# YaoChengTang/DecNet

Hardware: AMD Instinct MI355X
Metric: stereo pairs/sec at 960x540x192disp (hot path: stage-0 dense + SpaMat/SpaVar stages 1-3) (higher is better)
Workload: dtype f32 (bf16x3 on the bf16 matrix pipe); 1 GPU; BASELINE config 2: synthetic 960x540 (padded 972x540), max_disp 192->216: batch=8 synthetic pairs per GPU, feature maps of the 4-stage/scale-3 net, random-init CostRegNetNoDown(216); pairs_per_gpu=8, parallelism=dp1 (pairs sharded, all_gather of disparity maps)

## Files before the change

### decnet_amd/csrc/spamat_mfma.hip

```cpp
#include <stdlib.h>
#include <string.h>

#include <type_traits>

#include "common.h"


typedef float f32x4 __attribute__((ext_vector_type(4)));
typedef int i32x4 __attribute__((ext_vector_type(4)));
typedef __bf16 bf16x8 __attribute__((ext_vector_type(8)));

namespace {

enum { MODE_MAT = 0, MODE_VAR = 1, MODE_FUSED = 2 };

constexpr float NEG_BIG = -1.0e30f;
constexpr float LOG2E = 1.4426950408889634f;
constexpr int THREADS = 512, NWAVE = THREADS / 64;

__device__ __forceinline__ float fast_exp2(float x) { return __builtin_amdgcn_exp2f(x); }

__device__ __forceinline__ bool uniform_flag(bool f) { return __builtin_amdgcn_readfirstlane((int)f) != 0; }
template <bool SEL = true>
__device__ __forceinline__ float4 load4f(const float *__restrict__ safe, const float *__restrict__ row, int x, int W, bool ok) {
// ... 11 lines not shown
        if (x + 1 >= 0 && x + 1 < W) v.y = row[x + 1];
        if (x + 2 >= 0 && x + 2 < W) v.z = row[x + 2];
        if (x + 3 >= 0 && x + 3 < W) v.w = row[x + 3];
    }
    return v;
}
__device__ __forceinline__ float4 load4s(const float *__restrict__ row, int x, int W) {
    float4 v = make_float4(0.f, 0.f, 0.f, 0.f);
    if (x >= 0 && x < W) v.x = row[x];
    if (x + 1 >= 0 && x + 1 < W) v.y = row[x + 1];
    if (x + 2 >= 0 && x + 2 < W) v.z = row[x + 2];
    if (x + 3 >= 0 && x + 3 < W) v.w = row[x + 3];
    return v;
}

__device__ __forceinline__ int mask4_bits(const unsigned long long *__restrict__ rowbits, int x, int W) {
    if (x < 0 || x >= W) return 0;
    return (int)((rowbits[x >> 6] >> (x & 63)) & 15ull);
}

__device__ __forceinline__ int mask4_words(const unsigned *__restrict__ roww, int x, int W) {
    if (x < 0 || x >= W) return 0;
    return (int)((roww[x >> 5] >> (x & 31)) & 15u);
}

__device__ __forceinline__ void split3x8(const float (&x)[8], i32x4 &hi, i32x4 &mid, i32x4 &lo) {
    int h[8], m[8], l[8];
#pragma unroll
    for (int e = 0; e < 8; ++e) {
        h[e] = __float_as_int(x[e]) & 0xffff0000;
        const float r1 = x[e] - __int_as_float(h[e]);
        m[e] = __float_as_int(r1) & 0xffff0000;
        l[e] = __float_as_int(r1 - __int_as_float(m[e]));
    }
#pragma unroll
    for (int e = 0; e < 4; ++e) {
        hi[e] = __builtin_amdgcn_perm(h[2 * e + 1], h[2 * e], 0x07060302);
        mid[e] = __builtin_amdgcn_perm(m[2 * e + 1], m[2 * e], 0x07060302);
        lo[e] = __builtin_amdgcn_perm(l[2 * e + 1], l[2 * e], 0x07060302);
    }
}

__host__ __device__ inline int d16_pitch(int quads) { return quads + ((4 - quads) & 7); }
struct Layout {
    int SW, HALO, RP, Cq;
    int offR, offBX, offRK, offLM, offXL, offWT, total;
};
__host__ __device__ inline Layout make_layout(int C, int NT, int XT, bool d16 = false) {
    Layout l;
    l.SW = XT * 16;
    l.HALO = (NT - 1) * 16;
    l.Cq = (C + 3) & ~3;
    l.RP = ((l.HALO + l.SW + 31) & ~31) + 16;
    l.offR = 0;
    const int swh = ((XT + 1) / 2) * 16;
    const int rt = d16 ? 3 * ((C + 7) / 8) * 16 * (d16_pitch((l.HALO + swh) >> 2) + d16_pitch(swh >> 2)) : 0;
    l.offBX = l.offR + (l.Cq * l.RP > rt ? l.Cq * l.RP : rt);
    l.offRK = l.offBX + l.RP;
    l.offLM = l.offRK + l.RP + 4;
    l.offXL = l.offLM + l.SW + 16;
    l.offWT = l.offXL + l.SW;
    l.total = l.offWT + 32;
    return l;
}

__device__ __forceinline__ int wave_incl_scan(int v, int lane) {
#pragma unroll
    for (int o = 1; o < 64; o <<= 1) {
        int t = __shfl_up(v, o);
        if (lane >= o) v += t;
    }
    return v;
}

template <int M, int N, int STEP, class F>
__device__ __forceinline__ void live_tiles(int ntile, F &&f) {
    if constexpr (M < N) {
        if (STEP > 0 && M >= ntile) return;
        f(std::integral_constant<int, M>{});
        if constexpr (STEP == 2 && M + 1 < N) f(std::integral_constant<int, M + 1>{});
        live_tiles<M + (STEP > 1 ? STEP : 1), N, STEP>(ntile, f);
    }
}
template <int NTL, int MODE, int COMPACT>
__device__ __forceinline__ void softmax_passes(f32x4 (&acc)[NTL], int ntile, int D, int dl,
                                               const float *__restrict__ lds, int bias_off, int xr_off,
                                               int xlj, float mu_in,
                                               float &mx_o, float &S_o, float &mu_o, float &var_o,
                                               int m_lo = 0, int m_hi = 0) {
    constexpr int GS = COMPACT >= 2 ? 2 : COMPACT;
    int dlv = dl;
    asm volatile("" : "+v"(dlv));
    float mx0 = 0.000001f, mx1 = 0.000001f;
    (void)bias_off;
    int xo1 = xr_off;
    asm volatile("" : "+v"(xo1));
    const int *xp1 = reinterpret_cast<const int *>(lds) + xo1;
    const float xlf = (float)xlj, hD = 0.5f * (float)(D - 1), xlh = xlf - hD;
    live_tiles<0, NTL, GS>(ntile, [&](auto mc) {
        constexpr int m = decltype(mc)::value;
        {
            if (COMPACT >= 2) {
                if (COMPACT == 2 || m < m_lo || m >= m_hi) {
                    if (COMPACT == 3) asm volatile("" ::: "memory");
                    const float4 p = *reinterpret_cast<const float4 *>(xp1 + 16 * m);
                    acc[m][0] = fabsf(xlh - p.x) <= hD ? acc[m][0] : NEG_BIG;
                    acc[m][1] = fabsf(xlh - p.y) <= hD ? acc[m][1] : NEG_BIG;
                    acc[m][2] = fabsf(xlh - p.z) <= hD ? acc[m][2] : NEG_BIG;
                    acc[m][3] = fabsf(xlh - p.w) <= hD ? acc[m][3] : NEG_BIG;
                }
            } else if (COMPACT) {
                const int4 p = *reinterpret_cast<const int4 *>(xp1 + 16 * m);
                acc[m][0] = (unsigned)(xlj - p.x) < (unsigned)D ? acc[m][0] : NEG_BIG;
                acc[m][1] = (unsigned)(xlj - p.y) < (unsigned)D ? acc[m][1] : NEG_BIG;
                acc[m][2] = (unsigned)(xlj - p.z) < (unsigned)D ? acc[m][2] : NEG_BIG;
                acc[m][3] = (unsigned)(xlj - p.w) < (unsigned)D ? acc[m][3] : NEG_BIG;
            } else {
                if (m == 0 || 16 * m + 15 >= D) {
                    asm volatile("" ::: "memory");
#pragma unroll
                    for (int r = 0; r < 4; ++r) {
                        const int d = 16 * m + dlv - r;
                        acc[m][r] = (unsigned)d >= (unsigned)D ? NEG_BIG : acc[m][r];
                    }
                }
            }
            mx0 = fmaxf(fmaxf(mx0, acc[m][0]), acc[m][1]);
            mx1 = fmaxf(fmaxf(mx1, acc[m][2]), acc[m][3]);
        }
    });
    float mx = fmaxf(mx0, mx1);
    mx = fmaxf(mx, __shfl_xor(mx, 16));
    mx = fmaxf(mx, __shfl_xor(mx, 32));
    if (!COMPACT && MODE != MODE_MAT) {
        const float nmv = -mx * LOG2E;
        float Sa = 0.f, Sb = 0.f, T16a = 0.f, T16b = 0.f, Tt = 0.f;
#pragma unroll
        for (int m = 0; m < NTL; ++m) {
            if (m < ntile) {
                const float e0 = fast_exp2(fmaf(acc[m][0], LOG2E, nmv));
                const float e1 = fast_exp2(fmaf(acc[m][1], LOG2E, nmv));
                const float e2 = fast_exp2(fmaf(acc[m][2], LOG2E, nmv));
                const float e3 = fast_exp2(fmaf(acc[m][3], LOG2E, nmv));
                const float s4 = (e0 + e1) + (e2 + e3);
                const float t2 = fmaf(6.f, e3, fmaf(4.f, e2, e1 + e1));
                const float qq = fmaf(9.f, e3, fmaf(4.f, e2, e1));
                acc[m][0] = s4;
                acc[m][1] = t2;
                acc[m][2] = qq;
                if (m & 1) { Sb += s4; T16b = fmaf(s4, (float)(16 * m), T16b); }
                else { Sa += s4; T16a = fmaf(s4, (float)(16 * m), T16a); }
                Tt += t2;
            }
        }
        const float dlf = (float)dl;
        float Sl = Sa + Sb;
        float Tl = fmaf(dlf, Sl, fmaf(-0.5f, Tt, T16a + T16b));
        Sl += __shfl_xor(Sl, 16);
        Sl += __shfl_xor(Sl, 32);
        const float S = Sl + 0.000001f;
        float mu = mu_in;
        if (MODE != MODE_VAR) {
            Tl += __shfl_xor(Tl, 16);
            Tl += __shfl_xor(Tl, 32);
            mu = (Tl + 0.000001f) / S;
        }
        const float c0 = dlf - mu;
        float V0 = 0.f, V1 = 0.f;
#pragma unroll
        for (int m = 0; m < NTL; ++m) {
            if (m < ntile) {
                const float A = (float)(16 * m) + c0;
                const float u = fmaf(A, acc[m][0], -acc[m][1]);
                if (m & 1) V1 = fmaf(A, u, V1) + acc[m][2];
                else V0 = fmaf(A, u, V0) + acc[m][2];
            }
        }
        float Vl = V0 + V1;
        Vl += __shfl_xor(Vl, 16);
        Vl += __shfl_xor(Vl, 32);
        mx_o = mx; S_o = S; mu_o = mu; var_o = (Vl + 0.000001f) / S;
        return;
    }
    const float nm = -mx * LOG2E;
    float S0 = 0.f, S1 = 0.f, T0 = 0.f, T1 = 0.f;
    int xo2 = xr_off;
    asm volatile("" : "+v"(xo2));
    const int *xp2 = reinterpret_cast<const int *>(lds) + xo2;
    live_tiles<0, NTL, GS>(ntile, [&](auto mc) {
        constexpr int m = decltype(mc)::value;
        {
            int4 p;
            float4 pf;
            if (COMPACT >= 2) pf = *reinterpret_cast<const float4 *>(xp2 + 16 * m);
            else if (COMPACT) p = *reinterpret_cast<const int4 *>(xp2 + 16 * m);
#pragma unroll
            for (int r = 0; r < 4; r += 2) {
                float e0 = fast_exp2(fmaf(acc[m][r], LOG2E, nm));
                float e1 = fast_exp2(fmaf(acc[m][r + 1], LOG2E, nm));
                acc[m][r] = e0;
                acc[m][r + 1] = e1;
                S0 += e0;
                S1 += e1;
                if (MODE != MODE_VAR) {
                    if (COMPACT >= 2) {
                        T0 = fmaf(e0, xlf - (r == 0 ? pf.x : pf.z), T0);
                        T1 = fmaf(e1, xlf - (r == 0 ? pf.y : pf.w), T1);
                    } else if (COMPACT) {
                        T0 = fmaf(e0, (float)(xlj - (r == 0 ? p.x : p.z)), T0);
                        T1 = fmaf(e1, (float)(xlj - (r == 0 ? p.y : p.w)), T1);
                    } else {
                        T0 = fmaf(e0, (float)(16 * m - r), T0);
                        T1 = fmaf(e1, (float)(16 * m - r - 1), T1);
                    }
                }
            }
        }
    });
    const float dlf = (float)dl;
    float Sl = S0 + S1;
    float Tl = COMPACT ? T0 + T1 : fmaf(dlf, Sl, T0 + T1);
    Sl += __shfl_xor(Sl, 16);
    Sl += __shfl_xor(Sl, 32);
    const float S = Sl + 0.000001f;
    float mu = mu_in;
    if (MODE != MODE_VAR) {
        Tl += __shfl_xor(Tl, 16);
        Tl += __shfl_xor(Tl, 32);
        mu = (Tl + 0.000001f) / S;
    }
    float var = 0.f;
    if (MODE != MODE_MAT) {
        const float c0 = (COMPACT ? (float)xlj : dlf) - mu;
        float V0 = 0.f, V1 = 0.f;
        int xo3 = xr_off;
        asm volatile("" : "+v"(xo3));
        const int *xp3 = reinterpret_cast<const int *>(lds) + xo3;
        live_tiles<0, NTL, GS>(ntile, [&](auto mc) {
            constexpr int m = decltype(mc)::value;
            {
                int4 p;
                float4 pf;
                if (COMPACT >= 2) pf = *reinterpret_cast<const float4 *>(xp3 + 16 * m);
                else if (COMPACT) p = *reinterpret_cast<const int4 *>(xp3 + 16 * m);
#pragma unroll
                for (int r = 0; r < 4; r += 2) {
                    float d0, d1;
                    if (COMPACT >= 2) {
                        d0 = c0 - (r == 0 ? pf.x : pf.z);
                        d1 = c0 - (r == 0 ? pf.y : pf.w);
                    } else if (COMPACT) {
                        d0 = c0 - (float)(r == 0 ? p.x : p.z);
                        d1 = c0 - (float)(r == 0 ? p.y : p.w);
                    } else {
                        d0 = (float)(16 * m - r) + c0;
                        d1 = (float)(16 * m - r - 1) + c0;
                    }
                    V0 = fmaf(acc[m][r] * d0, d0, V0);
                    V1 = fmaf(acc[m][r + 1] * d1, d1, V1);
                }
            }
        });
        float Vl = V0 + V1;
        Vl += __shfl_xor(Vl, 16);
        Vl += __shfl_xor(Vl, 32);
        var = (Vl + 0.000001f) / S;
    }
    mx_o = mx; S_o = S; mu_o = mu; var_o = var;
}


__device__ __forceinline__ void dense16_loads8(float4 (&v)[8], const float *__restrict__ src, size_t plane, int g, int C,
                                               int x, int W, bool al) {
    if (al) {
        const bool whole = x + 3 < W;
#pragma unroll
        for (int c = 0; c < 8; ++c)
            v[c] = load4f<false>(src, src + (size_t)(8 * g + c) * plane, x, W, whole && 8 * g + c < C);
        __builtin_amdgcn_sched_barrier(0);
        if (__ballot(x < 0) != 0ull) {
#pragma unroll
            for (int c = 0; c < 8; ++c)
                if (x < 0) v[c] = make_float4(0.f, 0.f, 0.f, 0.f);
        }
        if (C & 7) {
#pragma unroll
            for (int c = 0; c < 8; ++c) {
                const bool ch = 8 * g + c < C;
                v[c] = make_float4(ch ? v[c].x : 0.f, ch ? v[c].y : 0.f, ch ? v[c].z : 0.f, ch ? v[c].w : 0.f);
            }
        }
        if ((W & 3) && x < W && !whole) {
#pragma unroll
            for (int c = 0; c < 8; ++c)
                v[c] = 8 * g + c < C ? load4s(src + (size_t)(8 * g + c) * plane, x, W) : make_float4(0.f, 0.f, 0.f, 0.f);
        }
    } else {
#pragma unroll
        for (int c = 0; c < 8; ++c)
            v[c] = 8 * g + c < C ? load4s(src + (size_t)(8 * g + c) * plane, x, W) : make_float4(0.f, 0.f, 0.f, 0.f);
    }
}

__device__ __forceinline__ void dense16_item_loads(float4 (&v)[8], int it, const float *__restrict__ lrow,
                                                   const float *__restrict__ rrow, size_t plane, int C, int W, int xs,
                                                   int SW, int HALO, int nRw) {
    const bool al = uniform_flag(((((uintptr_t)rrow) | ((uintptr_t)lrow) | ((uintptr_t)(plane * 4))) & 15) == 0);
    const int cg_n = (C + 7) >> 3, nqR = nRw >> 2, nqL = SW >> 2;
    const int nR_items = cg_n * nqR;
    const bool isL = it >= nR_items;
    const int k = isL ? it - nR_items : it, nq = isL ? nqL : nqR;
    const int g = k / nq, jq = k - g * nq;
    const float *src = isL ? lrow : rrow;
    const int x = isL ? xs + 4 * jq : xs - HALO + 4 * jq;
    dense16_loads8(v, src, plane, g, C, x, W, al);
}

template <int NT, int MODE, int CGT, bool PRE = false>
__device__ __forceinline__ void dense16_body(int *RT, const float *BX, const float *LM, const float *smem,
                                             const float *__restrict__ lrow, const float *__restrict__ rrow,
                                             const float *__restrict__ disparity, float *__restrict__ out,
                                             float *__restrict__ var_out, float *__restrict__ sum_sim,
                                             float *__restrict__ max_cost, size_t plane, size_t rowpix, int C, int W,
                                             int D, int xs, int XT, int SW, int HALO, int nRw, const float4 *pre = nullptr) {
    const int tid = threadIdx.x, lane = tid & 63, wave = tid >> 6;
    struct { int CG; } lo = {(C + 7) >> 3};
    const int PR = d16_pitch(nRw >> 2), PL = d16_pitch(SW >> 2);
    int *LT = RT + 3 * lo.CG * 16 * PR;
    {
        const bool al = uniform_flag(((((uintptr_t)rrow) | ((uintptr_t)lrow) | ((uintptr_t)(plane * 4))) & 15) == 0);
        const int cg_n = lo.CG, nqR = nRw >> 2, nqL = SW >> 2;
        const int nR_items = cg_n * nqR, n_items = nR_items + cg_n * nqL;
#pragma unroll 1
        for (int it = tid; it < n_items; it += THREADS) {
            const bool isL = it >= nR_items;
            const int k = isL ? it - nR_items : it, nq = isL ? nqL : nqR;
            const int g = k / nq, jq = k - g * nq;
            const float *src = isL ? lrow : rrow;
            const int x = isL ? xs + 4 * jq : xs - HALO + 4 * jq;
            float4 v[8];
            if (PRE && it == tid) {
#pragma unroll
                for (int c = 0; c < 8; ++c) v[c] = pre[c];
            } else {
                dense16_loads8(v, src, plane, g, C, x, W, al);
            }
            const int P = isL ? PL : PR;
            int *dst = (isL ? LT : RT) + (g * 4 * P + jq) * 4;
            const int tstride = cg_n * 16 * P;
#pragma unroll
            for (int pz = 0; pz < 4; ++pz) {
                float xv[8];
#pragma unroll
                for (int c = 0; c < 8; ++c) xv[c] = pz == 0 ? v[c].x : pz == 1 ? v[c].y : pz == 2 ? v[c].z : v[c].w;
                i32x4 th, tm, tl;
                split3x8(xv, th, tm, tl);
                *reinterpret_cast<i32x4 *>(dst + pz * 4 * P) = th;
                *reinterpret_cast<i32x4 *>(dst + tstride + pz * 4 * P) = tm;
                *reinterpret_cast<i32x4 *>(dst + 2 * tstride + pz * 4 * P) = tl;
            }
        }
    }
    __syncthreads();

    const int j = lane & 15, q = lane >> 4;
    const int dl = j - 4 * q;
    constexpr int CGB = CGT ? CGT : 1;
    const int cg_n = CGT ? CGT : lo.CG;
    const int tA_big = q >> 1, tA_small = q == 0 ? 0 : q == 2 ? 1 : 2;
    const int tB_big = q & 1, tB_small = q == 1 ? 0 : q == 3 ? 1 : 2;
    const int gsR = 16 * PR, gsL = 16 * PL;
    for (int xt = wave; xt < XT; xt += NWAVE) {
        const int x0 = xs + xt * 16;
        if (x0 >= W) break;
        const int x = x0 + j;
        const size_t pix = rowpix + x;
        const bool inside = x < W;
        const float rm = LM[xt * 16 + j];
        if (__ballot(rm != 0.f) == 0ull) {
            if (inside && q == 0) {
                if (MODE != MODE_VAR) out[pix] = 0.f;
                if (MODE != MODE_MAT) var_out[pix] = 0.f;
                sum_sim[pix] = 0.f;
                max_cost[pix] = 0.f;
            }
            continue;
        }
        f32x4 acc[NT];
#pragma unroll
        for (int m = 0; m < NT; ++m) {
            const float4 bz = *reinterpret_cast<const float4 *>(BX + (HALO + xt * 16) + 4 * q - 16 * m);
            acc[m] = f32x4{bz.x, bz.y, bz.z, bz.w};
        }
        const int sa = (j & 3) * PR + 4 * xt + (j >> 2), sb = (j & 3) * PL + 4 * xt + (j >> 2);
        const int *a_small = RT + (tA_small * cg_n * 4 * PR + sa) * 4;
        const int *a_big = RT + (tA_big * cg_n * 4 * PR + sa) * 4;
        const int *b_small = LT + (tB_small * cg_n * 4 * PL + sb) * 4;
        const int *b_big = LT + (tB_big * cg_n * 4 * PL + sb) * 4;
#pragma unroll
        for (int g = 0; g < CGB; ++g) {
            for (int gg = g; gg < cg_n; gg += CGB) {
                const i32x4 bs = *reinterpret_cast<const i32x4 *>(b_small + gg * gsL);
                const i32x4 bb = *reinterpret_cast<const i32x4 *>(b_big + gg * gsL);
#pragma unroll
                for (int m = 0; m < NT; ++m) {
                    const i32x4 av = *reinterpret_cast<const i32x4 *>(a_small + gg * gsR + (NT - 1 - m) * 16);
                    acc[m] = __builtin_amdgcn_mfma_f32_16x16x32_bf16(__builtin_bit_cast(bf16x8, av),
                                                                     __builtin_bit_cast(bf16x8, bs), acc[m], 0, 0, 0);
                }
#pragma unroll
                for (int m = 0; m < NT; ++m) {
                    const i32x4 av = *reinterpret_cast<const i32x4 *>(a_big + gg * gsR + (NT - 1 - m) * 16);
                    acc[m] = __builtin_amdgcn_mfma_f32_16x16x32_bf16(__builtin_bit_cast(bf16x8, av),
                                                                     __builtin_bit_cast(bf16x8, bb), acc[m], 0, 0, 0);
                }
            }
        }
        float mx, S, mu, var;
        const float mu_in = (MODE == MODE_VAR && inside) ? disparity[pix] : 0.f;
        softmax_passes<NT, MODE, 0>(acc, NT, D, dl, smem, 0, 0, 0, mu_in, mx, S, mu, var);
        if (inside && q == 0) {
            const bool on = rm != 0.f;
            if (MODE != MODE_VAR) out[pix] = on ? mu : 0.f;
            if (MODE != MODE_MAT) var_out[pix] = on ? var : 0.f;
            sum_sim[pix] = on ? S : 0.f;
            max_cost[pix] = on ? mx : 0.f;
        }
    }

}

template <int NT, int MODE, int KQ, int PPT, int NTHR, int CAP, int NTCMAX>
__device__ __forceinline__ int sparse_row_body(
    const float *__restrict__ ref, const float *__restrict__ tar, const float *__restrict__ rmask,
    const float *__restrict__ tmask, const float *__restrict__ disparity, float *__restrict__ out,
    float *__restrict__ var_out, float *__restrict__ sum_sim, float *__restrict__ max_cost, int C,
    int H, int W, int D, int row, int dense_pct, int mbits, int *fr_out = nullptr, int *fl_out = nullptr);
constexpr int MID_CAP = 640;

template <int NT, int MODE, int KQ, bool D16>
__device__ __forceinline__ void spamat_fwd_segment(
    const float *__restrict__ ref, const float *__restrict__ tar, const float *__restrict__ rmask,
    const float *__restrict__ tmask, const float *__restrict__ disparity, float *__restrict__ out,
    float *__restrict__ var_out, float *__restrict__ sum_sim, float *__restrict__ max_cost, int C,
    int H, int W, int D, int XT, int allow_compact, int marker, int seg, int row, int compact_pct, int mbits) {
    const float mark = marker ? sum_sim[(size_t)row * W + (size_t)seg * (XT * 16)] : -1.0f;
    if (marker && !(mark < 0.f))
        return;
    if constexpr (KQ == 2) {
        if (marker == 2 && mark == -2.0f) {
            if (sparse_row_body<NT, MODE, KQ, 4, THREADS, MID_CAP, NT + 1>(ref, tar, rmask, tmask, disparity, out, var_out,
                                                                          sum_sim, max_cost, C, H, W, D, row, 100,
                                                                          mbits) == 1)
                return;
            __syncthreads();
        }
    }
    extern __shared__ __attribute__((aligned(16))) float smem[];
    const Layout lo = make_layout(C, NT, XT, D16);
    float *Rs = smem + lo.offR;
    float *BX = smem + lo.offBX;
    int *XR = reinterpret_cast<int *>(BX);
    int *RK = reinterpret_cast<int *>(smem + lo.offRK);
    float *LM = smem + lo.offLM;
    int *RKL = reinterpret_cast<int *>(LM);
    int *XL = reinterpret_cast<int *>(smem + lo.offXL);
    int *WT = reinterpret_cast<int *>(smem + lo.offWT);
    const int SW = lo.SW, HALO = lo.HALO, RP = lo.RP;
    const int kq_n = KQ ? KQ : lo.Cq / 4;
    constexpr int KB = KQ ? KQ : 1;

    const int tid = threadIdx.x, lane = tid & 63, wave = tid >> 6;
    const int b = row / H, y = row - b * H;
    const int xs = seg * SW;
    const int nRw = HALO + SW;
    const size_t plane = (size_t)H * W;
    const float *lrow = ref + ((size_t)b * C * H + y) * W;
    const float *rrow = tar + ((size_t)b * C * H + y) * W;
    const float *trow = tmask + (size_t)row * W;
    const float *mrow = rmask + (size_t)row * W;
    const size_t rowpix = (size_t)row * W;
    const unsigned long long *tbits = reinterpret_cast<const unsigned long long *>(tmask) + (size_t)row * ((W + 63) >> 6);
    const unsigned long long *lbits = reinterpret_cast<const unsigned long long *>(rmask) + (size_t)row * ((W + 63) >> 6);

    unsigned mf_wr = 0, mf_wl = 0;
    if constexpr (D16) {
        if (mbits == 2) {
            const int q4 = tid * 4, xr_ = xs - HALO + q4, xl_ = xs + q4;
            const unsigned *hw = reinterpret_cast<const unsigned *>(max_cost + rowpix);
            mf_wr = hw[(q4 < nRw && xr_ >= 0 && xr_ < W) ? xr_ >> 5 : 0];
            mf_wl = hw[((W + 31) >> 5) + ((q4 < SW && xl_ < W) ? xl_ >> 5 : 0)];
        }
    }
    float4 d16_pre[D16 ? 8 : 1];
    if constexpr (D16) {
        const int xta = (XT + 1) / 2;
        const int n_items = ((C + 7) >> 3) * (((HALO + xta * 16) >> 2) + ((xta * 16) >> 2));
        if (tid < n_items) dense16_item_loads(d16_pre, tid, lrow, rrow, plane, C, W, xs, xta * 16, HALO, HALO + xta * 16);
    }
    const bool al_r = ((((uintptr_t)rrow) | ((uintptr_t)(plane * 4))) & 15) == 0;
    const int st_nq = nRw >> 2;
    const int st_rpp = THREADS / st_nq;
    const int st_r0 = tid / st_nq, st_jq = tid - st_r0 * st_nq;
    float4 st_v[D16 ? 1 : 8];
    float bfirst[(!D16 && KQ > 0) ? KQ : 1];
    if constexpr (!D16) {
        if (st_r0 < st_rpp) {
            const int x = xs - HALO + 4 * st_jq;
#pragma unroll
            for (int u = 0; u < 8; ++u) {
                const int c = st_r0 + u * st_rpp;
                st_v[u] = c < C ? load4_lanes(rrow + (size_t)c * plane, x, W, al_r) : make_float4(0.f, 0.f, 0.f, 0.f);
            }
        }
        if constexpr (KQ > 0) {
            const int jl = lane & 15, ql = lane >> 4;
            const int x = xs + wave * 16 + jl;
            const bool ok = wave < XT && x < W;
#pragma unroll
            for (int s = 0; s < KQ; ++s) bfirst[s] = (ok && 4 * s + ql < C) ? lrow[(size_t)(4 * s + ql) * plane + x] : 0.f;
        }
    }

    const int p4 = tid * 4;
    int fr = 0, fl = 0;
    {
        const bool alm = (((uintptr_t)trow) & 15) == 0 && (((uintptr_t)mrow) & 15) == 0;
        const bool almu = D16 && uniform_flag(alm && (W & 3) == 0);
        if (p4 < nRw) {
            const int x = xs - HALO + p4;
            if (mbits == 2) {
                if (D16) fr = (x >= 0 && x < W) ? (int)((mf_wr >> (x & 31)) & 15u) : 0;
                else fr = mask4_words(reinterpret_cast<const unsigned *>(max_cost + rowpix), x, W);
            } else if (mbits) {
                fr = mask4_bits(tbits, x, W);
            } else {
                float4 tv = almu ? load4f(trow, trow, x, W, true) : load4_lanes(trow, x, W, alm);
                fr = (tv.x != 0.f) | ((tv.y != 0.f) << 1) | ((tv.z != 0.f) << 2) | ((tv.w != 0.f) << 3);
            }
            float4 bv4;
            bv4.x = (fr & 1) ? 0.f : NEG_BIG;
            bv4.y = (fr & 2) ? 0.f : NEG_BIG;
            bv4.z = (fr & 4) ? 0.f : NEG_BIG;
            bv4.w = (fr & 8) ? 0.f : NEG_BIG;
            *reinterpret_cast<float4 *>(BX + p4) = bv4;
        }
        if (p4 < SW) {
            float4 mv;
            if (mbits) {
                if (D16 && mbits == 2) fl = (xs + p4 < W) ? (int)((mf_wl >> ((xs + p4) & 31)) & 15u) : 0;
                else fl = mbits == 2 ? mask4_words(reinterpret_cast<const unsigned *>(max_cost + rowpix) + ((W + 31) >> 5), xs + p4, W)
                                : mask4_bits(lbits, xs + p4, W);
                mv = make_float4((fl & 1) ? 1.f : 0.f, (fl & 2) ? 1.f : 0.f, (fl & 4) ? 1.f : 0.f, (fl & 8) ? 1.f : 0.f);
            } else {
                mv = almu ? load4f(mrow, mrow, xs + p4, W, true) : load4_lanes(mrow, xs + p4, W, alm);
                fl = (mv.x != 0.f) | ((mv.y != 0.f) << 1) | ((mv.z != 0.f) << 2) | ((mv.w != 0.f) << 3);
            }
            *reinterpret_cast<float4 *>(LM + p4) = mv;
        }
    }
    {
        const int ir = wave_incl_scan(__popc(fr), lane), il = wave_incl_scan(__popc(fl), lane);
        if (lane == 63) { WT[wave] = ir; WT[8 + wave] = il; }
    }

    int nR = 0, nL = 0;
    bool compact = false;
    if constexpr (D16) {
        __syncthreads();
#pragma unroll
        for (int w = 0; w < NWAVE; ++w) { nR += WT[w]; nL += WT[8 + w]; }
        const int validL = min(SW, W - xs);
        const int validR = min(W, xs + SW) - max(0, xs - HALO);
        compact = allow_compact && ((long)nL * nR * 100 < (long)validL * validR * compact_pct);
        if (!compact) {
            const int xta = (XT + 1) / 2, xtb = XT - xta;
            dense16_body<NT, MODE, (KQ + 1) / 2, true>(reinterpret_cast<int *>(Rs), BX, LM, smem, lrow, rrow, disparity, out,
                                                       var_out, sum_sim, max_cost, plane, rowpix, C, W, D, xs, xta, xta * 16,
                                                       HALO, HALO + xta * 16, d16_pre);
            if (xtb > 0 && xs + xta * 16 < W) {
                __syncthreads();
                dense16_body<NT, MODE, (KQ + 1) / 2>(reinterpret_cast<int *>(Rs), BX + xta * 16, LM + xta * 16, smem, lrow,
                                                     rrow, disparity, out, var_out, sum_sim, max_cost, plane, rowpix, C,
                                                     W, D, xs + xta * 16, xtb, xtb * 16, HALO, HALO + xtb * 16);
            }
            return;
        }
    }
    {
        const bool al = al_r;
        const int rpp = st_rpp;
        const int r0 = st_r0, jq = st_jq;
        if (r0 < rpp) {
            const int jj = 4 * jq, x = xs - HALO + jj;
            for (int c0 = r0; c0 < lo.Cq; c0 += 8 * rpp) {
                float4 v[8];
                if (!D16 && c0 == r0) {
#pragma unroll
                    for (int u = 0; u < 8; ++u) v[u] = st_v[D16 ? 0 : u];
                } else {
#pragma unroll
                    for (int u = 0; u < 8; ++u) {
                        const int c = c0 + u * rpp;
                        v[u] = c < C ? load4_lanes(rrow + (size_t)c * plane, x, W, al) : make_float4(0.f, 0.f, 0.f, 0.f);
                    }
                }
#pragma unroll
                for (int u = 0; u < 8; ++u) {
                    const int c = c0 + u * rpp;
                    if (c < lo.Cq) *reinterpret_cast<float4 *>(Rs + c * RP + jj) = v[u];
                }
            }
        }
        for (int c = tid; c < lo.Cq; c += THREADS) Rs[c * RP + RP - 1] = 0.f;
    }
    __syncthreads();

    const int validL = min(SW, W - xs);
    const int validR = min(W, xs + SW) - max(0, xs - HALO);
    if constexpr (!D16) {
#pragma unroll
        for (int w = 0; w < NWAVE; ++w) { nR += WT[w]; nL += WT[8 + w]; }
        compact = allow_compact && ((long)nL * nR * 100 < (long)validL * validR * compact_pct);
    }

    const int j = lane & 15, q = lane >> 4;

    if constexpr (!D16) if (!compact) {
        const int dl = j - 4 * q;
        float bv[KQ <= 6 ? KB : 1], bcur[KB];
        float rm = 0.f;
        auto fetch_left = [&](int xt, float (&dst)[KB]) {
            const int x = xs + xt * 16 + j;
            const bool ok = xt < XT && x < W;
            if (KQ) {
#pragma unroll
                for (int s = 0; s < KQ; ++s)
                    dst[s] = (ok && 4 * s + q < C) ? lrow[(size_t)(4 * s + q) * plane + x] : 0.f;
            }
        };
        constexpr bool PREF = KQ <= 6;
        if constexpr (PREF && KQ > 0) {
#pragma unroll
            for (int s = 0; s < KB; ++s) bv[s] = bfirst[s];
        } else if constexpr (PREF) {
            fetch_left(wave, bv);
        }
        for (int xt = wave; xt < XT; xt += NWAVE) {
            const int x0 = xs + xt * 16;
            if (x0 >= W) break;
            const int x = x0 + j;
            const size_t pix = rowpix + x;
            const bool inside = x < W;
            rm = LM[xt * 16 + j];
            if constexpr (PREF) {
#pragma unroll
                for (int s = 0; s < KB; ++s) bcur[s] = bv[s];
                fetch_left(xt + NWAVE, bv);
            } else if (KQ > 0 && xt == wave) {
#pragma unroll
                for (int s = 0; s < KB; ++s) bcur[s] = bfirst[KQ > 0 ? s : 0];
            } else {
                fetch_left(xt, bcur);
            }
            if (__ballot(rm != 0.f) == 0ull) {
                if (inside && q == 0) {
                    if (MODE != MODE_VAR) out[pix] = 0.f;
// ... 82 lines not shown
    while (S > 16 && (long)S * nL > 24L * validL) S >>= 1;
    __syncthreads();
    constexpr int NTC = NT + 1;
    while (S > 16) {
        int bad = 0;
        for (int g = tid; g * S < SW; g += THREADS) {
            const int jlo = max(0, g * S + HALO - (D - 1)), jhi = min(nRw - 1, g * S + HALO + S - 1);
            if (RK[jhi + 1] - RK[jlo] > 16 * NTC - 15) bad = 1;
        }
        if (!__syncthreads_or(bad)) break;
        S >>= 1;
    }

    for (int p = tid; p < validL; p += THREADS) {
        if (RKL[p + 1] == RKL[p]) {
            const size_t pix = rowpix + xs + p;
            if (MODE != MODE_VAR) out[pix] = 0.f;
            if (MODE != MODE_MAT) var_out[pix] = 0.f;
            sum_sim[pix] = 0.f;
            max_cost[pix] = 0.f;
        }
    }

    const int ngroups = (SW + S - 1) / S;
    for (int g = wave; g < ngroups; g += NWAVE) {
        const int gx = g * S;
        const int e0 = __builtin_amdgcn_readfirstlane(RKL[gx]), e1 = __builtin_amdgcn_readfirstlane(RKL[min(gx + S, SW)]);
        if (e1 == e0) continue;
        const int jlo = max(0, gx + HALO - (D - 1)), jhi = min(nRw - 1, gx + HALO + S - 1);
        const int r_lo = __builtin_amdgcn_readfirstlane(RK[jlo]), r_hi = __builtin_amdgcn_readfirstlane(RK[jhi + 1]);
        const int t0 = r_lo >> 4;
        const int ntile = r_hi > r_lo ? ((r_hi - 1) >> 4) - t0 + 1 : 0;
        for (int e = e0; e < e1; e += 16) {
            const bool act = e + j < e1;
            const int xl = XL[act ? e + j : e1 - 1];
            const int x = xs + xl;
            const size_t pix = rowpix + x;
            float bcur[KB];
            if (KQ) {
#pragma unroll
                for (int s = 0; s < KQ; ++s)
                    bcur[s] = (act && 4 * s + q < C) ? lrow[(size_t)(4 * s + q) * plane + x] : 0.f;
            }
            f32x4 acc[NTC];
            const int *xa = XR + 16 * t0 + j;
            live_tiles<0, NTC, 1>(ntile, [&](auto mc) {
                constexpr int m = decltype(mc)::value;
                {
                    const float *ap = Rs + q * RP + xa[16 * m];
                    f32x4 a4 = f32x4{0.f, 0.f, 0.f, 0.f};
                    if (KQ) {
#pragma unroll
                        for (int s = 0; s < KQ; ++s)
                            a4 = __builtin_amdgcn_mfma_f32_16x16x4f32(ap[4 * s * RP], bcur[s], a4, 0, 0, 0);
                    } else {
                        const float *bp = lrow + (size_t)q * plane + x;
                        for (int s = 0; s < kq_n; ++s) {
                            const float lv = (act && 4 * s + q < C) ? bp[(size_t)4 * s * plane] : 0.f;
                            a4 = __builtin_amdgcn_mfma_f32_16x16x4f32(ap[4 * s * RP], lv, a4, 0, 0, 0);
                        }
                    }
                    acc[m] = a4;
                }
            });
            float mx, Ssum, mu, var;
            const float mu_in = (MODE == MODE_VAR && act) ? disparity[pix] : 0.f;
            softmax_passes<NTC, MODE, 1>(acc, ntile, D, 0, smem, 0, lo.offBX + 16 * t0 + 4 * q, xl + HALO, mu_in,
                                         mx, Ssum, mu, var);
            if (act && q == 0) {
                if (MODE != MODE_VAR) out[pix] = mu;
                if (MODE != MODE_MAT) var_out[pix] = var;
                sum_sim[pix] = Ssum;
                max_cost[pix] = mx;
            }
        }
    }
}

template <int NT, int MODE, int KQ, bool D16>
__global__ __launch_bounds__(THREADS, (KQ > 6 ? 2 : 4)) void spamat_fwd_mfma(
    const float *__restrict__ ref, const float *__restrict__ tar, const float *__restrict__ rmask,
    const float *__restrict__ tmask, const float *__restrict__ disparity, float *__restrict__ out,
    float *__restrict__ var_out, float *__restrict__ sum_sim, float *__restrict__ max_cost, int C,
    int H, int W, int D, int segs_per_row, int XT, int allow_compact, int marker, int compact_pct, int mbits) {
    spamat_fwd_segment<NT, MODE, KQ, D16>(ref, tar, rmask, tmask, disparity, out, var_out, sum_sim, max_cost, C, H, W,
                                          D, XT, allow_compact, marker, blockIdx.x % segs_per_row,
                                          blockIdx.x / segs_per_row, compact_pct, mbits);
}

constexpr int SP_THREADS = 256, SP_CAP = 256;
constexpr size_t sparse_row_words(int kq, int ppt, int nthr, int cap) {
    return (size_t)(cap + 32) + 2 * (size_t)(nthr * ppt / 2 + 2) + cap + 32 + 2 * (size_t)4 * kq * (cap + 16);
}

template <int NT, int MODE, int KQ, int PPT, int NTHR, int CAP, int NTCMAX>
__device__ __forceinline__ int sparse_row_body(
    const float *__restrict__ ref, const float *__restrict__ tar, const float *__restrict__ rmask,
    const float *__restrict__ tmask, const float *__restrict__ disparity, float *__restrict__ out,
    float *__restrict__ var_out, float *__restrict__ sum_sim, float *__restrict__ max_cost, int C,
    int H, int W, int D, int row, int dense_pct, int mbits, int *fr_out, int *fl_out) {
    constexpr int CQ = 4 * KQ, NTC = NT + 1 < NTCMAX ? NT + 1 : NTCMAX;
    constexpr int SP_NWAVE_ = NTHR / 64, SP_FP_ = CAP + 16;
    extern __shared__ __attribute__((aligned(16))) float smem[];
    constexpr int NPX = NTHR * PPT, RKW = NPX / 2 + 2;
    constexpr int offXR = 0, offRK = CAP + 32, offRKL = offRK + RKW, offXL = offRKL + RKW,
                  offWT = offXL + CAP, offRF = offWT + 32, offLF = offRF + CQ * SP_FP_;
    float *XR = smem + offXR;
    unsigned short *RK = reinterpret_cast<unsigned short *>(smem + offRK);
    unsigned short *RKL = reinterpret_cast<unsigned short *>(smem + offRKL);
    int *XL = reinterpret_cast<int *>(smem) + offXL;
    int *WT = reinterpret_cast<int *>(smem) + offWT;
    float *RF = smem + offRF, *LF = smem + offLF;

    const int tid = threadIdx.x, lane = tid & 63, wave = tid >> 6;
    const int b = row / H, y = row - b * H;
    const size_t plane = (size_t)H * W, rowpix = (size_t)row * W;
    const float *lrow = ref + ((size_t)b * C * H + y) * W;
    const float *rrow = tar + ((size_t)b * C * H + y) * W;
    const float *trow = tmask + rowpix, *mrow = rmask + rowpix;

    constexpr bool ALL = CAP > 256 && PPT == 4;
    const int p4 = tid * PPT;
    float4 lv[ALL ? CQ : 1], rv[ALL ? CQ : 1];
    if constexpr (ALL) {
        const bool alf = ((W & 3) == 0) && ((((uintptr_t)lrow) | ((uintptr_t)rrow) | ((uintptr_t)(plane * 4))) & 15) == 0;
#pragma unroll
        for (int c = 0; c < CQ; ++c) {
            const bool ok = p4 < W && c < C;
            lv[c] = ok ? load4_lanes(lrow + (size_t)c * plane, p4, W, alf) : make_float4(0.f, 0.f, 0.f, 0.f);
            rv[c] = ok ? load4_lanes(rrow + (size_t)c * plane, p4, W, alf) : make_float4(0.f, 0.f, 0.f, 0.f);
        }
    }
    int fr = 0, fl = 0;
    {
        const bool alm = ((W & 3) == 0) && ((((uintptr_t)trow) | ((uintptr_t)mrow)) & 15) == 0;
#pragma unroll
        for (int u = 0; u < PPT; u += 4) {
            if (p4 + u < W) {
                if (mbits == 2) {
                    const unsigned *hw = reinterpret_cast<const unsigned *>(max_cost + rowpix);
                    fr |= mask4_words(hw, p4 + u, W) << u;
                    fl |= mask4_words(hw + ((W + 31) >> 5), p4 + u, W) << u;
                } else if (mbits) {
                    const int wpr = (W + 63) >> 6;
                    fr |= mask4_bits(reinterpret_cast<const unsigned long long *>(tmask) + (size_t)row * wpr, p4 + u, W) << u;
                    fl |= mask4_bits(reinterpret_cast<const unsigned long long *>(rmask) + (size_t)row * wpr, p4 + u, W) << u;
                } else {
                    const float4 tv = load4_lanes(trow, p4 + u, W, alm), mv = load4_lanes(mrow, p4 + u, W, alm);
                    fr |= ((tv.x != 0.f) | ((tv.y != 0.f) << 1) | ((tv.z != 0.f) << 2) | ((tv.w != 0.f) << 3)) << u;
                    fl |= ((mv.x != 0.f) | ((mv.y != 0.f) << 1) | ((mv.z != 0.f) << 2) | ((mv.w != 0.f) << 3)) << u;
                }
            }
        }
    }
    if (fr_out) { *fr_out = fr; *fl_out = fl; }
    const int cr = __popc(fr), cl = __popc(fl);
    const int ir = wave_incl_scan(cr, lane), il = wave_incl_scan(cl, lane);
    if (lane == 63) { WT[wave] = ir; WT[8 + wave] = il; }
    __syncthreads();
    int nR = 0, nL = 0, baseR = 0, baseL = 0;
#pragma unroll
    for (int w = 0; w < SP_NWAVE_; ++w) {
        if (w < wave) { baseR += WT[w]; baseL += WT[8 + w]; }
        nR += WT[w];
        nL += WT[8 + w];
    }
    nR = __builtin_amdgcn_readfirstlane(nR);
    nL = __builtin_amdgcn_readfirstlane(nL);
    if ((long)nL * nR * 100 >= (long)W * W * dense_pct) return 0;
    if (nL > CAP || nR > CAP) return (nL <= MID_CAP && nR <= MID_CAP) ? 2 : 0;
// ... 137 lines not shown
                if (MODE != MODE_VAR) *reinterpret_cast<float4 *>(out + pix) = make_float4(r[0][0], r[0][1], r[0][2], r[0][3]);
                if (MODE != MODE_MAT) *reinterpret_cast<float4 *>(var_out + pix) = make_float4(r[1][0], r[1][1], r[1][2], r[1][3]);
                *reinterpret_cast<float4 *>(sum_sim + pix) = make_float4(r[2][0], r[2][1], r[2][2], r[2][3]);
                *reinterpret_cast<float4 *>(max_cost + pix) = make_float4(r[3][0], r[3][1], r[3][2], r[3][3]);
            } else {
#pragma unroll
                for (int k = 0; k < 4; ++k) {
                    if (p4 + u + k < W) {
                        if (MODE != MODE_VAR) out[pix + k] = r[0][k];
                        if (MODE != MODE_MAT) var_out[pix + k] = r[1][k];
                        sum_sim[pix + k] = r[2][k];
                        max_cost[pix + k] = r[3][k];
                    }
                }
            }
        }
    }
    return 1;
}

template <int NT, int MODE, int KQ, int PPT>
__global__ __launch_bounds__(SP_THREADS, PPT == 4 ? 6 : 5) void spamat_fwd_sparse(
    const float *__restrict__ ref, const float *__restrict__ tar, const float *__restrict__ rmask,
    const float *__restrict__ tmask, const float *__restrict__ disparity, float *__restrict__ out,
    float *__restrict__ var_out, float *__restrict__ sum_sim, float *__restrict__ max_cost, int C,
    int H, int W, int D, int seg_w, int dense_pct, int mbits, int handover) {
    const int row = blockIdx.x;
    int fr = 0, fl = 0;
    const int rc = sparse_row_body<NT, MODE, KQ, PPT, SP_THREADS, SP_CAP, 8>(ref, tar, rmask, tmask, disparity, out, var_out,
                                                                            sum_sim, max_cost, C, H, W, D, row, dense_pct, mbits,
                                                                            &fr, &fl);
    if (rc != 1) {
        const size_t rowpix = (size_t)row * W;
        const float mark = rc == 2 ? -2.0f : -1.0f;
        for (int x = threadIdx.x * seg_w; x < W; x += SP_THREADS * seg_w) sum_sim[rowpix + x] = mark;
        if (handover) {
            extern __shared__ __attribute__((aligned(16))) float smem[];
            unsigned *wb = reinterpret_cast<unsigned *>(smem);
            const int nw = (W + 31) >> 5, p4 = threadIdx.x * PPT;
            __syncthreads();
            for (int i = threadIdx.x; i < 2 * nw; i += SP_THREADS) wb[i] = 0u;
            __syncthreads();
            if (p4 < W) {
                if (fr) atomicOr(&wb[p4 >> 5], (unsigned)fr << (p4 & 31));
                if (fl) atomicOr(&wb[nw + (p4 >> 5)], (unsigned)fl << (p4 & 31));
            }
            __syncthreads();
            for (int i = threadIdx.x; i < 2 * nw; i += SP_THREADS) reinterpret_cast<unsigned *>(max_cost + rowpix)[i] = wb[i];
        }
    }
}

template <int NT, int KQ>
int launch_nt(int mode, const float *ref, const float *tar, const float *rmask, const float *tmask,
              const float *disparity, float *out, float *var_out, float *sum_sim, float *max_cost,
              int B, int C, int H, int W, int D, int allow_compact, int mbits, hipStream_t stream) {
    const int xt_row = ceil_div(W, 16);
    static const int dense_fp32 = [] { const char *e = getenv("DECNET_SPAMAT_DENSE"); return e && !strcmp(e, "fp32"); }();
    const bool d16 = KQ == 2 && !dense_fp32;
    auto bytes = [&](int xt) { return (size_t)4 * make_layout(C, NT, xt, d16).total; };
    const size_t budget2 = (DECNET_LDS_BYTES - 2048) / 2, budget1 = DECNET_LDS_BYTES - 1024;
    int XT = xt_row > 64 ? ceil_div(xt_row, ceil_div(xt_row, 64)) : xt_row;
    if (bytes(XT) > budget2) {
        int segs = ceil_div(xt_row, XT) + 1;
        while (segs < xt_row && bytes(ceil_div(xt_row, segs)) > budget2) ++segs;
        int xt2 = ceil_div(xt_row, segs);
        if (bytes(xt2) <= budget2) XT = xt2;
        else {
            while (XT > 1 && bytes(XT) > budget1) --XT;
        }
    }
    XT = (XT + 1) & ~1;
    if (XT > 64) XT = 64;
    const size_t lds = bytes(XT);
    if (lds > budget1 || make_layout(C, NT, XT, d16).RP > 2048) return DECNET_ERR_UNSUPPORTED;
    const int segs = ceil_div(xt_row, XT);
    dim3 block(THREADS);
    constexpr int compact_pct = 35;
    constexpr int sparse_pct = 45;
    dim3 grid((unsigned)((size_t)B * H * segs));
    int marker = allow_compact && KQ == 2 && W <= 2048;
    static const bool mid_off = [] { const char *e = getenv("DECNET_SPAMAT_MID"); return e && atoi(e) == 0; }();
    size_t lds_launch = lds;
    static const bool handover_off = [] { const char *e = getenv("DECNET_SPAMAT_HANDOVER"); return e && atoi(e) == 0; }();
    const int handover = (KQ > 0 && KQ <= 6 && marker && segs == 1 && !mbits && 2 * ((W + 31) / 32) <= W && !handover_off) ? 1 : 0;
    if (KQ == 2 && marker && segs == 1 && !mid_off) {
        const size_t need = 4 * sparse_row_words(KQ, 4, THREADS, MID_CAP);
        if (need <= budget2 + 8192) {
            marker = 2;
            if (need > lds_launch) lds_launch = need;
        }
    }
    if constexpr (KQ > 0 && KQ <= 6) if (marker) {
        const int ppt = W <= 1024 ? 4 : 8;
        const size_t slds = 4 * sparse_row_words(KQ, ppt, SP_THREADS, SP_CAP);
#define LAUNCHS(M, P)                                                                              \
    do {                                                                                           \
        if (slds > 64 * 1024) {                                                                    \
            hipError_t e = hipFuncSetAttribute((const void *)spamat_fwd_sparse<NT, M, (KQ ? KQ : 1), P>, \
                                               hipFuncAttributeMaxDynamicSharedMemorySize, (int)slds); \
            if (e != hipSuccess) return (int)e;                                                    \
        }                                                                                          \
        hipLaunchKernelGGL((spamat_fwd_sparse<NT, M, (KQ ? KQ : 1), P>), dim3((unsigned)(B * H)),  \
                           dim3(SP_THREADS), slds, stream, ref, tar, rmask, tmask, disparity, out, \
                           var_out, sum_sim, max_cost, C, H, W, D, XT * 16, sparse_pct, mbits, handover); \
    } while (0)
#define LAUNCHSP(M)                                                                                \
    do {                                                                                           \
        if (ppt == 4) LAUNCHS(M, 4);                                                               \
        else LAUNCHS(M, 8);                                                                        \
    } while (0)
        if (mode == MODE_MAT) LAUNCHSP(MODE_MAT);
        else if (mode == MODE_VAR) LAUNCHSP(MODE_VAR);
        else LAUNCHSP(MODE_FUSED);
#undef LAUNCHSP
#undef LAUNCHS
        int rc = decnet_launch_status();
        if (rc) return rc;
    }
#define LAUNCH1(M, DD)                                                                             \
    do {                                                                                           \
        if (lds_launch > 64 * 1024) {                                                              \
            hipError_t e = hipFuncSetAttribute((const void *)spamat_fwd_mfma<NT, M, KQ, DD>,       \
                                               hipFuncAttributeMaxDynamicSharedMemorySize, (int)lds_launch); \
            if (e != hipSuccess) return (int)e;                                                    \
        }                                                                                          \
        hipLaunchKernelGGL((spamat_fwd_mfma<NT, M, KQ, DD>), grid, block, lds_launch, stream, ref, tar, rmask, \
                           tmask, disparity, out, var_out, sum_sim, max_cost, C, H, W, D, segs, XT, \
                           allow_compact, marker, compact_pct, handover ? 2 : mbits);              \
    } while (0)
#define LAUNCH(M)                                                                                  \
    do {                                                                                           \
        if constexpr (KQ == 2) {                                                                   \
            if (d16) LAUNCH1(M, true);                                                             \
            else LAUNCH1(M, false);                                                                \
        } else {                                                                                   \
            LAUNCH1(M, false);                                                                     \
        }                                                                                          \
    } while (0)
    if (mode == MODE_MAT) LAUNCH(MODE_MAT);
    else if (mode == MODE_VAR) LAUNCH(MODE_VAR);
    else LAUNCH(MODE_FUSED);
#undef LAUNCH1
#undef LAUNCH
    return decnet_launch_status();
}

template <int NT>
int launch_kq(int mode, const float *ref, const float *tar, const float *rmask, const float *tmask,
              const float *disparity, float *out, float *var_out, float *sum_sim, float *max_cost,
              int B, int C, int H, int W, int D, int allow_compact, int mbits, hipStream_t stream) {
#define GO(K)                                                                                      \
    return launch_nt<NT, K>(mode, ref, tar, rmask, tmask, disparity, out, var_out, sum_sim,        \
                            max_cost, B, C, H, W, D, allow_compact, mbits, stream)
    if (C <= 8 && C > 4) GO(2);
    if (C <= 24 && C > 20) GO(6);
    if (C <= 72 && C > 68) GO(18);
    GO(0);
#undef GO
}

}

int decnet_mfma_forward(int mode, const float *ref, const float *tar, const float *rmask,
                        const float *tmask, const float *disparity, float *out, float *var_out,
                        float *sum_sim, float *max_cost, int B, int C, int H, int W, int max_disp,
                        int allow_compact, int mbits, hipStream_t stream) {
    const int D = max_disp;
    const int need = D <= 1 ? 1 : (D - 1 + 15) / 16 + 1;
#define GO(N)                                                                                     \
    return launch_kq<N>(mode, ref, tar, rmask, tmask, disparity, out, var_out, sum_sim, max_cost, \
                        B, C, H, W, D, allow_compact, mbits, stream)
    if (need <= 3) GO(3);
    if (need <= 6) GO(6);
    if (need <= 8) GO(8);
    if (need <= 11) GO(11);
    if (need <= 15) GO(15);
    if (need <= 18) GO(18);
    return DECNET_ERR_UNSUPPORTED;
#undef GO
}
```

Before: 5145 pairs/s.

## Skip out-of-range disparity tiles near the left image edge in dense16 path

Near the left border, pixels at x0 can only match disparities up to x0, so the dense16 body now computes only the first min(NT, x0/16+1) disparity tiles (MFMA, bias init and softmax moments) via a gated variant, and skips loading right-image halo chunks with negative x. Wave-to-tile assignment is also reversed on alternate rounds to balance the now-uneven per-tile cost across waves. An env var DECNET_SPAMAT_RAMP=0 disables it. This adds a second instantiation of the tile body, which raises code size and may affect register pressure, and skipped halo loads leave LDS entries unwritten that must never be read.

```diff
diff --git a/decnet_amd/csrc/spamat_mfma.hip b/decnet_amd/csrc/spamat_mfma.hip
--- a/decnet_amd/csrc/spamat_mfma.hip
+++ b/decnet_amd/csrc/spamat_mfma.hip
@@ -117,13 +117,14 @@
         live_tiles<M + (STEP > 1 ? STEP : 1), N, STEP>(ntile, f);
     }
 }
-template <int NTL, int MODE, int COMPACT>
+template <int NTL, int MODE, int COMPACT, bool GATED = false>
 __device__ __forceinline__ void softmax_passes(f32x4 (&acc)[NTL], int ntile, int D, int dl,
                                                const float *__restrict__ lds, int bias_off, int xr_off,
                                                int xlj, float mu_in,
                                                float &mx_o, float &S_o, float &mu_o, float &var_o,
                                                int m_lo = 0, int m_hi = 0) {
-    constexpr int GS = COMPACT >= 2 ? 2 : COMPACT;
+    static_assert(!GATED || COMPACT == 0, "GATED is the dense callers' switch");
+    constexpr int GS = COMPACT >= 2 ? 2 : (COMPACT || GATED) ? 1 : 0;
     int dlv = dl;
     asm volatile("" : "+v"(dlv));
     float mx0 = 0.000001f, mx1 = 0.000001f;
@@ -170,9 +171,9 @@
     if (!COMPACT && MODE != MODE_MAT) {
         const float nmv = -mx * LOG2E;
         float Sa = 0.f, Sb = 0.f, T16a = 0.f, T16b = 0.f, Tt = 0.f;
-#pragma unroll
-        for (int m = 0; m < NTL; ++m) {
-            if (m < ntile) {
+        auto moments = [&](auto mc) {
+            constexpr int m = decltype(mc)::value;
+            {
                 const float e0 = fast_exp2(fmaf(acc[m][0], LOG2E, nmv));
                 const float e1 = fast_exp2(fmaf(acc[m][1], LOG2E, nmv));
                 const float e2 = fast_exp2(fmaf(acc[m][2], LOG2E, nmv));
@@ -187,6 +188,28 @@
                 else { Sa += s4; T16a = fmaf(s4, (float)(16 * m), T16a); }
                 Tt += t2;
             }
+        };
+        if constexpr (GATED) {
+            live_tiles<0, NTL, 1>(ntile, moments);
+        } else {
+#pragma unroll
+            for (int m = 0; m < NTL; ++m) {
+                if (m < ntile) {
+                    const float e0 = fast_exp2(fmaf(acc[m][0], LOG2E, nmv));
+                    const float e1 = fast_exp2(fmaf(acc[m][1], LOG2E, nmv));
+                    const float e2 = fast_exp2(fmaf(acc[m][2], LOG2E, nmv));
+                    const float e3 = fast_exp2(fmaf(acc[m][3], LOG2E, nmv));
+                    const float s4 = (e0 + e1) + (e2 + e3);
+                    const float t2 = fmaf(6.f, e3, fmaf(4.f, e2, e1 + e1));
+                    const float qq = fmaf(9.f, e3, fmaf(4.f, e2, e1));
+                    acc[m][0] = s4;
+                    acc[m][1] = t2;
+                    acc[m][2] = qq;
+                    if (m & 1) { Sb += s4; T16b = fmaf(s4, (float)(16 * m), T16b); }
+                    else { Sa += s4; T16a = fmaf(s4, (float)(16 * m), T16a); }
+                    Tt += t2;
+                }
+            }
         }
         const float dlf = (float)dl;
         float Sl = Sa + Sb;
@@ -202,13 +225,23 @@
         }
         const float c0 = dlf - mu;
         float V0 = 0.f, V1 = 0.f;
-#pragma unroll
-        for (int m = 0; m < NTL; ++m) {
-            if (m < ntile) {
+        if constexpr (GATED) {
+            live_tiles<0, NTL, 1>(ntile, [&](auto mc) {
+                constexpr int m = decltype(mc)::value;
                 const float A = (float)(16 * m) + c0;
                 const float u = fmaf(A, acc[m][0], -acc[m][1]);
                 if (m & 1) V1 = fmaf(A, u, V1) + acc[m][2];
                 else V0 = fmaf(A, u, V0) + acc[m][2];
+            });
+        } else {
+#pragma unroll
+            for (int m = 0; m < NTL; ++m) {
+                if (m < ntile) {
+                    const float A = (float)(16 * m) + c0;
+                    const float u = fmaf(A, acc[m][0], -acc[m][1]);
+                    if (m & 1) V1 = fmaf(A, u, V1) + acc[m][2];
+                    else V0 = fmaf(A, u, V0) + acc[m][2];
+                }
             }
         }
         float Vl = V0 + V1;
@@ -357,7 +390,8 @@
                                              const float *__restrict__ disparity, float *__restrict__ out,
                                              float *__restrict__ var_out, float *__restrict__ sum_sim,
                                              float *__restrict__ max_cost, size_t plane, size_t rowpix, int C, int W,
-                                             int D, int xs, int XT, int SW, int HALO, int nRw, const float4 *pre = nullptr) {
+                                             int D, int xs, int XT, int SW, int HALO, int nRw, int ramp,
+                                             const float4 *pre = nullptr) {
     const int tid = threadIdx.x, lane = tid & 63, wave = tid >> 6;
     struct { int CG; } lo = {(C + 7) >> 3};
     const int PR = d16_pitch(nRw >> 2), PL = d16_pitch(SW >> 2);
@@ -373,6 +407,7 @@
             const int g = k / nq, jq = k - g * nq;
             const float *src = isL ? lrow : rrow;
             const int x = isL ? xs + 4 * jq : xs - HALO + 4 * jq;
+            if (ramp && !isL && x < 0) continue;
             float4 v[8];
             if (PRE && it == tid) {
 #pragma unroll
@@ -405,7 +440,43 @@
     const int tA_big = q >> 1, tA_small = q == 0 ? 0 : q == 2 ? 1 : 2;
     const int tB_big = q & 1, tB_small = q == 1 ? 0 : q == 3 ? 1 : 2;
     const int gsR = 16 * PR, gsL = 16 * PL;
-    for (int xt = wave; xt < XT; xt += NWAVE) {
+    auto left_tile = [&](auto gated, int nlive, int xt, int Dt, float mu_in, float &mx, float &S, float &mu, float &var) {
+        constexpr int G = decltype(gated)::value ? 1 : 0;
+        f32x4 acc[NT];
+        live_tiles<0, NT, G>(nlive, [&](auto mc) {
+            constexpr int m = decltype(mc)::value;
+            const float4 bz = *reinterpret_cast<const float4 *>(BX + (HALO + xt * 16) + 4 * q - 16 * m);
+            acc[m] = f32x4{bz.x, bz.y, bz.z, bz.w};
+        });
+        const int sa = (j & 3) * PR + 4 * xt + (j >> 2), sb = (j & 3) * PL + 4 * xt + (j >> 2);
+        const int *a_small = RT + (tA_small * cg_n * 4 * PR + sa) * 4;
+        const int *a_big = RT + (tA_big * cg_n * 4 * PR + sa) * 4;
+        const int *b_small = LT + (tB_small * cg_n * 4 * PL + sb) * 4;
+        const int *b_big = LT + (tB_big * cg_n * 4 * PL + sb) * 4;
+#pragma unroll
+        for (int g = 0; g < CGB; ++g) {
+            for (int gg = g; gg < cg_n; gg += CGB) {
+                const i32x4 bs = *reinterpret_cast<const i32x4 *>(b_small + gg * gsL);
+                const i32x4 bb = *reinterpret_cast<const i32x4 *>(b_big + gg * gsL);
+                live_tiles<0, NT, G>(nlive, [&](auto mc) {
+                    constexpr int m = decltype(mc)::value;
+                    const i32x4 av = *reinterpret_cast<const i32x4 *>(a_small + gg * gsR + (NT - 1 - m) * 16);
+                    acc[m] = __builtin_amdgcn_mfma_f32_16x16x32_bf16(__builtin_bit_cast(bf16x8, av),
+                                                                     __builtin_bit_cast(bf16x8, bs), acc[m], 0, 0, 0);
+                });
+                live_tiles<0, NT, G>(nlive, [&](auto mc) {
+                    constexpr int m = decltype(mc)::value;
+                    const i32x4 av = *reinterpret_cast<const i32x4 *>(a_big + gg * gsR + (NT - 1 - m) * 16);
+                    acc[m] = __builtin_amdgcn_mfma_f32_16x16x32_bf16(__builtin_bit_cast(bf16x8, av),
+                                                                     __builtin_bit_cast(bf16x8, bb), acc[m], 0, 0, 0);
+                });
+            }
+        }
+        softmax_passes<NT, MODE, 0, G != 0>(acc, nlive, Dt, dl, smem, 0, 0, 0, mu_in, mx, S, mu, var);
+    };
+    for (int xk = 0; xk < XT; xk += NWAVE) {
+        const int xt = xk + ((ramp && (xk & NWAVE)) ? NWAVE - 1 - wave : wave);
+        if (xt >= XT) break;
         const int x0 = xs + xt * 16;
         if (x0 >= W) break;
         const int x = x0 + j;
@@ -421,39 +492,13 @@
             }
             continue;
         }
-        f32x4 acc[NT];
-#pragma unroll
-        for (int m = 0; m < NT; ++m) {
-            const float4 bz = *reinterpret_cast<const float4 *>(BX + (HALO + xt * 16) + 4 * q - 16 * m);
-            acc[m] = f32x4{bz.x, bz.y, bz.z, bz.w};
-        }
-        const int sa = (j & 3) * PR + 4 * xt + (j >> 2), sb = (j & 3) * PL + 4 * xt + (j >> 2);
-        const int *a_small = RT + (tA_small * cg_n * 4 * PR + sa) * 4;
-        const int *a_big = RT + (tA_big * cg_n * 4 * PR + sa) * 4;
-        const int *b_small = LT + (tB_small * cg_n * 4 * PL + sb) * 4;
-        const int *b_big = LT + (tB_big * cg_n * 4 * PL + sb) * 4;
-#pragma unroll
-        for (int g = 0; g < CGB; ++g) {
-            for (int gg = g; gg < cg_n; gg += CGB) {
-                const i32x4 bs = *reinterpret_cast<const i32x4 *>(b_small + gg * gsL);
-                const i32x4 bb = *reinterpret_cast<const i32x4 *>(b_big + gg * gsL);
-#pragma unroll
-                for (int m = 0; m < NT; ++m) {
-                    const i32x4 av = *reinterpret_cast<const i32x4 *>(a_small + gg * gsR + (NT - 1 - m) * 16);
-                    acc[m] = __builtin_amdgcn_mfma_f32_16x16x32_bf16(__builtin_bit_cast(bf16x8, av),
-                                                                     __builtin_bit_cast(bf16x8, bs), acc[m], 0, 0, 0);
-                }
-#pragma unroll
-                for (int m = 0; m < NT; ++m) {
-                    const i32x4 av = *reinterpret_cast<const i32x4 *>(a_big + gg * gsR + (NT - 1 - m) * 16);
-                    acc[m] = __builtin_amdgcn_mfma_f32_16x16x32_bf16(__builtin_bit_cast(bf16x8, av),
-                                                                     __builtin_bit_cast(bf16x8, bb), acc[m], 0, 0, 0);
-                }
-            }
-        }
         float mx, S, mu, var;
         const float mu_in = (MODE == MODE_VAR && inside) ? disparity[pix] : 0.f;
-        softmax_passes<NT, MODE, 0>(acc, NT, D, dl, smem, 0, 0, 0, mu_in, mx, S, mu, var);
+        const int nlive = __builtin_amdgcn_readfirstlane(ramp ? min(NT, (x0 >> 4) + 1) : NT);
+        int Dt = D;
+        asm volatile("" : "+s"(Dt));
+        if (nlive == NT) left_tile(std::false_type{}, NT, xt, Dt, mu_in, mx, S, mu, var);
+        else left_tile(std::true_type{}, nlive, xt, Dt, mu_in, mx, S, mu, var);
         if (inside && q == 0) {
             const bool on = rm != 0.f;
             if (MODE != MODE_VAR) out[pix] = on ? mu : 0.f;
@@ -478,7 +523,7 @@
     const float *__restrict__ ref, const float *__restrict__ tar, const float *__restrict__ rmask,
     const float *__restrict__ tmask, const float *__restrict__ disparity, float *__restrict__ out,
     float *__restrict__ var_out, float *__restrict__ sum_sim, float *__restrict__ max_cost, int C,
-    int H, int W, int D, int XT, int allow_compact, int marker, int seg, int row, int compact_pct, int mbits) {
+    int H, int W, int D, int XT, int allow_compact, int marker, int seg, int row, int compact_pct, int mbits, int ramp) {
     const float mark = marker ? sum_sim[(size_t)row * W + (size_t)seg * (XT * 16)] : -1.0f;
     if (marker && !(mark < 0.f))
         return;
@@ -612,12 +657,12 @@
             const int xta = (XT + 1) / 2, xtb = XT - xta;
             dense16_body<NT, MODE, (KQ + 1) / 2, true>(reinterpret_cast<int *>(Rs), BX, LM, smem, lrow, rrow, disparity, out,
                                                        var_out, sum_sim, max_cost, plane, rowpix, C, W, D, xs, xta, xta * 16,
-                                                       HALO, HALO + xta * 16, d16_pre);
+                                                       HALO, HALO + xta * 16, ramp, d16_pre);
             if (xtb > 0 && xs + xta * 16 < W) {
                 __syncthreads();
                 dense16_body<NT, MODE, (KQ + 1) / 2>(reinterpret_cast<int *>(Rs), BX + xta * 16, LM + xta * 16, smem, lrow,
                                                      rrow, disparity, out, var_out, sum_sim, max_cost, plane, rowpix, C,
-                                                     W, D, xs + xta * 16, xtb, xtb * 16, HALO, HALO + xtb * 16);
+                                                     W, D, xs + xta * 16, xtb, xtb * 16, HALO, HALO + xtb * 16, ramp);
             }
             return;
         }
@@ -866,10 +911,10 @@
     const float *__restrict__ ref, const float *__restrict__ tar, const float *__restrict__ rmask,
     const float *__restrict__ tmask, const float *__restrict__ disparity, float *__restrict__ out,
     float *__restrict__ var_out, float *__restrict__ sum_sim, float *__restrict__ max_cost, int C,
-    int H, int W, int D, int segs_per_row, int XT, int allow_compact, int marker, int compact_pct, int mbits) {
+    int H, int W, int D, int segs_per_row, int XT, int allow_compact, int marker, int compact_pct, int mbits, int ramp) {
     spamat_fwd_segment<NT, MODE, KQ, D16>(ref, tar, rmask, tmask, disparity, out, var_out, sum_sim, max_cost, C, H, W,
                                           D, XT, allow_compact, marker, blockIdx.x % segs_per_row,
-                                          blockIdx.x / segs_per_row, compact_pct, mbits);
+                                          blockIdx.x / segs_per_row, compact_pct, mbits, ramp);
 }
 
 constexpr int SP_THREADS = 256, SP_CAP = 256;
@@ -1173,6 +1218,7 @@
     int marker = allow_compact && KQ == 2 && W <= 2048;
     static const bool mid_off = [] { const char *e = getenv("DECNET_SPAMAT_MID"); return e && atoi(e) == 0; }();
     size_t lds_launch = lds;
+    static const int ramp = [] { const char *e = getenv("DECNET_SPAMAT_RAMP"); return (e && atoi(e) == 0) ? 0 : 1; }();
     static const bool handover_off = [] { const char *e = getenv("DECNET_SPAMAT_HANDOVER"); return e && atoi(e) == 0; }();
     const int handover = (KQ > 0 && KQ <= 6 && marker && segs == 1 && !mbits && 2 * ((W + 31) / 32) <= W && !handover_off) ? 1 : 0;
     if (KQ == 2 && marker && segs == 1 && !mid_off) {
@@ -1218,7 +1264,7 @@
         }                                                                                          \
         hipLaunchKernelGGL((spamat_fwd_mfma<NT, M, KQ, DD>), grid, block, lds_launch, stream, ref, tar, rmask, \
                            tmask, disparity, out, var_out, sum_sim, max_cost, C, H, W, D, segs, XT, \
-                           allow_compact, marker, compact_pct, handover ? 2 : mbits);              \
+                           allow_compact, marker, compact_pct, handover ? 2 : mbits, ramp);        \
     } while (0)
 #define LAUNCH(M)                                                                                  \
     do {                                                                                           \
```

Measured after the change: 5164 pairs/s, median of 6. Within noise of the previous version (+0.4%).
